# ratan-lab/indelMINER

Measured on AMD Instinct MI355X. Metric: reads/sec through split-read realign+cluster; VCF diff-clean vs reference, higher is better.
Workload: dtype u8/int32; 1 GPU; BASELINE configs[1]: synthetic 1.0 Mb contig per GPU, 100 bp PE reads at 30x, seeded 1-50 bp indels every ~2 kb, BWA-like S/I/D emission; -k 6 -g 0 -s 1000 -n 10 -q 10; pipeline_depth=4, hip_graph=True, parallelism=contig-sharded x1

## Files before the change

### indelminer_amd/csrc/im_rg.hpp

```cpp

#pragma once

#include "im_device.hpp"

namespace im {
namespace {

__device__ __forceinline__ uint32_t ld_u32(const uint8_t* p) { uint32_t v; __builtin_memcpy(&v, p, 4); return v; }

struct RecView {
    const uint8_t* p;
    uint32_t len;
    int32_t tid, pos, mtid, mpos, isize, l_seq;
    uint32_t l_qname, mapq, n_cigar, flag;
    uint32_t o_cigar, o_seq, o_aux;
    uint32_t cig[4];
    bool ok;
};

constexpr int kAuxWin = 24;

__device__ __forceinline__ RecView view_record(const uint8_t* raw, uint32_t off, uint32_t end)
{
    RecView r;
    r.p = raw + off; r.len = end - off; r.ok = false;
    r.tid = r.pos = r.mtid = r.mpos = r.isize = r.l_seq = 0;
    r.l_qname = r.mapq = r.n_cigar = r.flag = 0; r.o_cigar = r.o_seq = r.o_aux = 0;
    r.cig[0] = r.cig[1] = r.cig[2] = r.cig[3] = 0;
    if (end < off || r.len < 32u) return r;
    const uint32_t* c = reinterpret_cast<const uint32_t*>(r.p);
    r.tid = (int32_t)c[0]; r.pos = (int32_t)c[1];
    const uint32_t w2 = c[2], w3 = c[3];
    r.l_qname = w2 & 255u; r.mapq = (w2 >> 8) & 255u;
    r.n_cigar = w3 & 0xFFFFu; r.flag = w3 >> 16;
    r.l_seq = (int32_t)c[4]; r.mtid = (int32_t)c[5]; r.mpos = (int32_t)c[6]; r.isize = (int32_t)c[7];
    if (r.l_seq < 0) return r;
    r.o_cigar = 32u + r.l_qname;
    r.o_seq = r.o_cigar + 4u * r.n_cigar;
    const bool no_qual = (w2 >> 16) == 0xFFFFu;
    const uint64_t o_aux = (uint64_t)r.o_seq + (((uint64_t)r.l_seq + 1u) >> 1) + (no_qual ? 0ull : (uint64_t)r.l_seq);
    if (o_aux > r.len) return r;
    r.o_aux = (uint32_t)o_aux;
    r.ok = true;
    return r;
}

__device__ __forceinline__ int aux_size(uint32_t t)
{
    switch (t) {
    case 'A': case 'c': case 'C': return 1;
    case 's': case 'S': return 2;
    case 'i': case 'I': case 'f': return 4;
    case 'd': return 8;
    default: return 0;
    }
}

struct AuxWin { uint32_t* lds; uint32_t o0; };
__device__ __forceinline__ uint32_t rec_byte(const RecView& r, const AuxWin& w, uint32_t o)
{
    const uint32_t d = o - w.o0;
    return d < (uint32_t)kAuxWin ? reinterpret_cast<const uint8_t*>(w.lds)[d] : r.p[o];
}
__device__ __forceinline__ void aux_slide(const RecView& r, AuxWin& w, uint32_t o)
{
    w.o0 = o;
#pragma unroll
    for (int k = 0; k < kAuxWin / 4; k++) w.lds[k] = ld_u32(r.p + o + 4u * k);
}
__device__ __forceinline__ uint32_t walk_byte(const RecView& r, AuxWin& w, uint32_t o)
{
    if (o - w.o0 >= (uint32_t)kAuxWin) aux_slide(r, w, o);
    return reinterpret_cast<const uint8_t*>(w.lds)[o - w.o0];
}
__device__ __forceinline__ void aux_cover(const RecView& r, AuxWin& w, uint32_t o, uint32_t need)
{
    if (!(o >= w.o0 && o + need <= w.o0 + (uint32_t)kAuxWin)) aux_slide(r, w, o);
}

__device__ __forceinline__ void find_rg_mq(const RecView& r, AuxWin& w, uint32_t& o_rg, uint32_t& o_mq)
{
    o_rg = 0; o_mq = 0;
    uint32_t s = r.o_aux;
    const uint32_t end = r.len;
    while (s + 4u <= end) {
        aux_cover(r, w, s, 8u);
        const uint32_t t0 = rec_byte(r, w, s), t1 = rec_byte(r, w, s + 1), type = rec_byte(r, w, s + 2);
        if (t0 == 'R' && t1 == 'G' && !o_rg) o_rg = s + 2u;
        if (t0 == 'M' && t1 == 'Q' && !o_mq) o_mq = s + 2u;
        if (o_rg && o_mq) return;
        s += 3u;
        if (type == 'Z' || type == 'H') { while (s < end && walk_byte(r, w, s)) s++; s++; }
        else if (type == 'B') {
            if (s + 5u > end) return;
            const int sz = aux_size(rec_byte(r, w, s));
            const uint32_t cnt = rec_byte(r, w, s + 1) | (rec_byte(r, w, s + 2) << 8) | (rec_byte(r, w, s + 3) << 16) | (rec_byte(r, w, s + 4) << 24);
            const uint64_t ns = (uint64_t)s + 5u + (uint64_t)sz * cnt;
            if (ns > end) return;
            s = (uint32_t)ns;
        } else {
            const int sz = aux_size(type);
            if (sz == 0) return;
            s += (uint32_t)sz;
        }
    }
}

struct RgView {
    const int32_t* bin_start; const int32_t* name_off; const int32_t* name_len; const int32_t* range_max; const uint8_t* names;
};
__device__ __forceinline__ RgView rg_view(const uint8_t* blob, int32_t n)
{
    RgView v;
    const int32_t* w = reinterpret_cast<const int32_t*>(blob);
    const int32_t m = n > 0 ? n : 1;
    v.bin_start = w; v.name_off = w + 20; v.name_len = w + 20 + m; v.range_max = w + 20 + 2 * m;
    v.names = blob + 4 * (20 + 3 * m);
    return v;
}

template <typename NameAt>
__device__ __forceinline__ bool rg_lookup(const RgView& T, NameAt name_at, uint32_t len, int32_t& range_max)
{
    uint32_t h = 5381u;
    for (int i = (int)len - 1; i >= 0; i--) h += (h << 5) + (uint32_t)(int32_t)(int8_t)name_at((uint32_t)i);
    const uint32_t bin = h & 15u;
    bool hit = false;
    for (int32_t e = T.bin_start[bin]; e < T.bin_start[bin + 1]; e++) {
        const uint32_t el = (uint32_t)T.name_len[e];
        if (el < len) continue;
        const uint8_t* en = T.names + T.name_off[e];
        bool same = true;
        for (uint32_t i = 0; i < len && same; i++) same = en[i] == name_at(i);
        if (same) { hit = true; range_max = T.range_max[e]; }
    }
    return hit;
}

__device__ __forceinline__ bool rg_tag_range(const RecView& r, AuxWin& w, uint32_t o_rg, const RgView& T, int32_t& range_max)
{
    const uint32_t type = rec_byte(r, w, o_rg);
    bool ok = type == 'Z' || type == 'H';
    if (ok) {
        uint32_t len = 0;
        while (o_rg + 1u + len < r.len) {
            const uint32_t o = o_rg + 1u + len;
            if (o - w.o0 >= (uint32_t)kAuxWin && w.o0 != o_rg) aux_slide(r, w, o_rg);
            if (!rec_byte(r, w, o)) break;
            len++;
        }
        const uint32_t o_name = o_rg + 1u;
        ok = rg_lookup(T, [&](uint32_t k) { return rec_byte(r, w, o_name + k); }, len, range_max);
    }
    return ok;
}

constexpr int kRgLds = 2048;

}
}
```

### indelminer_amd/csrc/im_triage.hip

```cpp

#include "im_device.hpp"
#include "im_rg.hpp"
#include "im_wave.hpp"

#ifdef IM_STAMPS
constexpr int kTriStampCap = 32768;
__device__ unsigned long long im_tri_stamp_rec[kTriStampCap][8];
#define IM_TRI_STAMP_DECL unsigned long long tri_t_[6]; tri_t_[0] = __builtin_amdgcn_s_memtime(); \
                          tri_t_[1] = tri_t_[2] = tri_t_[3] = tri_t_[4] = tri_t_[5] = tri_t_[0];
#define IM_TRI_STAMP(k, v) do { asm volatile("" :: "v"(v)); tri_t_[k] = __builtin_amdgcn_s_memtime(); } while (0)
#define IM_TRI_STAMP_OUT(lane) do { if ((lane) < 6) { const int l_ = (lane); \
        im_tri_stamp_rec[blockIdx.x % kTriStampCap][l_] = l_ == 0 ? tri_t_[0] : l_ == 1 ? tri_t_[1] : l_ == 2 ? tri_t_[2] : l_ == 3 ? tri_t_[3] : l_ == 4 ? tri_t_[4] : tri_t_[5]; } } while (0)
#else
#define IM_TRI_STAMP_DECL
#define IM_TRI_STAMP(k, v)
#define IM_TRI_STAMP_OUT(lane)
#endif

namespace im {
namespace {

constexpr int kTriBlock = 256;
constexpr int kTriGroup = 32;

__device__ __forceinline__ uint32_t ld_u16(const uint8_t* p) { uint16_t v; __builtin_memcpy(&v, p, 2); return v; }


__device__ __forceinline__ uint32_t cigar_word(const RecView& r, uint32_t k)
{
    return k == 0u ? r.cig[0] : k == 1u ? r.cig[1] : k == 2u ? r.cig[2] : k == 3u ? r.cig[3] : ld_u32(r.p + r.o_cigar + 4u * k);
}

__device__ __forceinline__ int32_t aux_int(const RecView& r, const AuxWin& w, uint32_t o)
{
    const uint32_t type = rec_byte(r, w, o);
    if (o + 1u >= r.len) return 0;
    const uint32_t b0 = rec_byte(r, w, o + 1);
    switch (type) {
    case 'c': return (int32_t)(int8_t)b0;
    case 'C': return (int32_t)b0;
    case 's': return (o + 3u <= r.len) ? (int32_t)(int16_t)(b0 | (rec_byte(r, w, o + 2) << 8)) : 0;
    case 'S': return (o + 3u <= r.len) ? (int32_t)(b0 | (rec_byte(r, w, o + 2) << 8)) : 0;
    case 'i': case 'I':
        return (o + 5u <= r.len) ? (int32_t)(b0 | (rec_byte(r, w, o + 2) << 8) | (rec_byte(r, w, o + 3) << 16) | (rec_byte(r, w, o + 4) << 24)) : 0;
    default: return 0;
    }
}


__device__ __forceinline__ bool reaches_new_readaln(const RecView& r)
{
    const uint32_t f = r.flag;
    return r.ok && !(f & (0x100u | 0x200u | 0x400u | 0x800u)) && (f & 0x1u) && (f & 0x2u) && !(f & (0x4u | 0x8u)) && r.tid == r.mtid;
}

__device__ __forceinline__ uint32_t bases_in_cigar_reach(const RecView& r)
{
    uint64_t qtot = 0;
    for (uint32_t i = 0; i < r.n_cigar; i++) {
        const uint32_t cw = cigar_word(r, i), op = cw & 15u;
        if (op == 0u || op == 1u || op == 4u || op == 7u || op == 8u) qtot += cw >> 4;
    }
    const uint64_t avail = 2ull * (r.len - r.o_seq);
    return (uint32_t)(qtot < avail ? qtot : avail);
}

__device__ __forceinline__ uint32_t good_codes(uint32_t x)
{
    const uint32_t c = x - ((x >> 1) & 0x77777777u) - ((x >> 2) & 0x33333333u) - ((x >> 3) & 0x11111111u);
    return (c >> 2) | (c & ~(c >> 1));
}

__device__ __forceinline__ uint32_t first_refused(const uint4& x)
{
    const uint32_t w[4] = { x.x, x.y, x.z, x.w };
    for (uint32_t k = 0; k < 4u; k++) {
        const uint32_t bad = ~good_codes(w[k]) & 0x11111111u;
        if (bad) return 8u * k + ((uint32_t)__builtin_ctz(((bad & 0x0F0F0F0Fu) << 4) | ((bad >> 4) & 0x0F0F0F0Fu)) >> 2);
    }
    return 32u;
}

__device__ __forceinline__ bool all_good(const uint4& x)
{
    return ((good_codes(x.x) & good_codes(x.y) & good_codes(x.z) & good_codes(x.w)) & 0x11111111u) == 0x11111111u;
}

struct BaseSweep {
    uint4 x[8];
    uint32_t lm[8];
    int shift;
};

__device__ __forceinline__ void sweep_issue(BaseSweep& S, const uint8_t* raw, uint32_t so, uint32_t lim, int lane)
{
    S.shift = __ballot(lim > 128u) != 0ull ? 3 : 2;
    const uint32_t sub = (uint32_t)lane & ((1u << S.shift) - 1u);
    const int grp = lane >> S.shift, per_pass = 64 >> S.shift;
#pragma unroll
    for (int j = 0; j < 8; j++) {
        S.lm[j] = 0u; S.x[j] = make_uint4(0x11111111u, 0x11111111u, 0x11111111u, 0x11111111u);
        if (j < (1 << S.shift)) {
            const int src = per_pass * j + grp;
            S.lm[j] = (uint32_t)__shfl((int)lim, src);
            const uint32_t so_j = (uint32_t)__shfl((int)so, src);
            __builtin_memcpy(&S.x[j], raw + (32u * sub < S.lm[j] ? so_j + 16u * sub : 0u), 16);
        }
    }
}

__device__ __forceinline__ void sweep_finish(const BaseSweep& S, const uint8_t* raw, uint32_t so, uint32_t lim, uint32_t* s_fb, int lane)
{
    const uint32_t lanes = 1u << S.shift, sub = (uint32_t)lane & (lanes - 1u);
    const int grp = lane >> S.shift, per_pass = 64 >> S.shift;
#pragma unroll
    for (int j = 0; j < 8; j++) {
        if (j < (1 << S.shift) && 32u * sub < S.lm[j] && !all_good(S.x[j])) {
            const uint32_t idx = 32u * sub + first_refused(S.x[j]);
            if (idx < S.lm[j]) atomicMin(&s_fb[per_pass * j + grp], idx);
        }
    }
    if (__ballot(lim > 256u) != 0ull) {
        for (int j = 0; j < 8; j++) {
            const int src = per_pass * j + grp;
            const uint32_t lm = (uint32_t)__shfl((int)lim, src), so_j = (uint32_t)__shfl((int)so, src);
            for (uint32_t first = 256u + 32u * sub; first < lm; first += 256u) {
                uint4 x; __builtin_memcpy(&x, raw + so_j + (first >> 1), 16);
                if (!all_good(x)) { const uint32_t idx = first + first_refused(x); if (idx < lm) atomicMin(&s_fb[src], idx); }
            }
        }
    }
}

struct Verdict {
    uint32_t cls;
    bool revcomp;
    int32_t range_max;
};

__device__ __forceinline__ Verdict classify(const RecView& r, AuxWin w, const im_triage_params& tp, const RgView& T,
                                            bool generic_ok, int32_t generic_range, uint32_t fb)
{
    Verdict v; v.cls = IM_REC_SKIP; v.revcomp = false; v.range_max = 0;
    if (!r.ok) { v.cls = IM_REC_ERR_LIMIT; return v; }
    const uint32_t flag = r.flag;
    if (flag & (0x100u | 0x200u | 0x400u | 0x800u)) return v;
    const bool aligned = !(flag & 0x4u), mate_aligned = !(flag & 0x8u);
    const bool proper = (flag & 0x2u) != 0, is_rc = (flag & 0x10u) != 0, mate_rc = (flag & 0x20u) != 0;
    if (!(flag & 0x1u)) return v;
    if (aligned && mate_aligned && r.tid != r.mtid) return v;
    v.cls = IM_REC_COUNTED;

    uint32_t o_rg, o_mq;
    find_rg_mq(r, w, o_rg, o_mq);
    if (tp.defer_ranges) {
        if (o_rg) { const uint32_t type = rec_byte(r, w, o_rg); if (!(type == 'Z' || type == 'H')) { v.cls = IM_REC_ERR_RG; return v; } }
        v.range_max = 0;
    } else if (!o_rg) {
        if (!generic_ok) { v.cls = IM_REC_ERR_RG; return v; }
        v.range_max = generic_range;
    } else {
        if (!rg_tag_range(r, w, o_rg, T, v.range_max)) { v.cls = IM_REC_ERR_RG; return v; }
    }

    if (aligned && !mate_aligned) return v;
    if (!aligned && mate_aligned) {
        int32_t mmq = (int32_t)r.mapq;
        if (o_mq) {
            aux_cover(r, w, o_mq, 5u);
            const uint32_t t = rec_byte(r, w, o_mq);
            if (!(t == 'I' || t == 'i' || t == 'C' || t == 'c' || t == 'S' || t == 's')) { v.cls = IM_REC_ERR_MQ; return v; }
            mmq = aux_int(r, w, o_mq);
        }
        if (mmq >= tp.qthreshold) { v.cls = IM_REC_CAND_UNMAPPED; v.revcomp = !mate_rc; }
        return v;
    }
    if (aligned && mate_aligned && proper) {
        const uint32_t lim = bases_in_cigar_reach(r);
        if (fb >= lim) {
            fb = 0xFFFFFFFFu;
            for (uint32_t j = (uint32_t)r.l_seq; j < lim; j++) {
                const uint32_t code = (r.p[r.o_seq + (j >> 1)] >> ((~j & 1u) << 2)) & 15u;
                if (!(code == 1u || code == 2u || code == 4u || code == 8u || code == 15u)) { fb = j; break; }
            }
        }
        uint32_t ndel = 0, nins = 0, nclip = 0; bool three = false;
        uint64_t q = 0;
        for (uint32_t i = 0; i < r.n_cigar; i++) {
            const uint32_t cw = cigar_word(r, i), op = cw & 15u;
            if (op == 3u || op == 5u || op == 6u || op > 8u) { v.cls = (uint64_t)fb < q ? IM_REC_ERR_BASE : IM_REC_ERR_CIGAR; return v; }
            if (op == 0u || op == 1u || op == 4u || op == 7u || op == 8u) q += cw >> 4;
            ndel += op == 2u; nins += op == 1u; nclip += op == 4u;
            if (op == 4u && ((!is_rc && i == r.n_cigar - 1u) || (is_rc && i == 0u))) three = true;
        }
        if (fb != 0xFFFFFFFFu) { v.cls = IM_REC_ERR_BASE; return v; }
        if (ndel + nins + nclip == 0u) return v;
        if ((nclip == 0u || (nclip == 1u && three)) && ndel == 0u && nins == 0u) return v;
        if (o_mq) aux_cover(r, w, o_mq, 5u);
        const int32_t mmq = o_mq ? aux_int(r, w, o_mq) : (int32_t)r.mapq;
        if (mmq >= tp.qthreshold) { v.cls = IM_REC_CAND_PROPER; v.revcomp = is_rc == mate_rc; }
        return v;
    }
    if (aligned && mate_aligned && !proper) {
        const int64_t a = r.isize < 0 ? -(int64_t)r.isize : (int64_t)r.isize;
        const uint32_t a32 = (uint32_t)(r.isize < 0 ? -r.isize : r.isize);
        if (a > (int64_t)v.range_max && a32 < tp.maxpedelsize && is_rc != mate_rc) v.cls = IM_REC_PE;
        return v;
    }
    return v;
}

struct TriageArgs {
    im_dev_records recs;
    im_dev_cands out;
    im_triage_params tp;
    RefDev ref;
    RgTable rg;
    int32_t* depth_diff;
    uint32_t* info;
    int32_t* rmax;
    uint2* blk;
    uint2* wg_base;
    uint32_t* seq_at;
    int32_t* chunk_base;
};

__device__ __forceinline__ uint32_t padded4(int32_t l) { return ((uint32_t)l + 3u) & ~3u; }

constexpr int kClsBlock = 64;
constexpr int kClsLdsBudget = 6400;
constexpr int kDepthWin = 1024;
constexpr int kClsRgLds = 448;
static_assert(kTriBlock % kClsBlock == 0 && kTriGroup % (kTriBlock / kClsBlock) == 0, "an emit workgroup's classify blocks lie in one group");
static_assert(kClsBlock < 512, "a workgroup's candidate, counted and error counts take nine bits each of its packed word");
static_assert(kClsBlock * kAuxWin + kClsBlock * 4 + kDepthWin * 4 + kClsRgLds <= kClsLdsBudget, "classify must fit the hole a realign wave leaves");

__device__ __forceinline__ void wave_lds_order() { __builtin_amdgcn_fence(__ATOMIC_ACQ_REL, "wavefront"); }

__global__ __launch_bounds__(kClsBlock, 6) void triage_classify_kernel(TriageArgs A)
{
    __shared__ uint32_t s_aux[kClsBlock][kAuxWin / 4];
    __shared__ uint32_t s_rg[kClsRgLds / 4];
    __shared__ int32_t s_dd[kDepthWin];
    __shared__ uint32_t s_fb[kClsBlock];
    const int lane = threadIdx.x;
    IM_TRI_STAMP_DECL
    const int64_t i = (int64_t)blockIdx.x * kClsBlock + lane;
    if (A.depth_diff) {
        int4* z = reinterpret_cast<int4*>(s_dd);
#pragma unroll
        for (int k = 0; k < kDepthWin / 4 / kClsBlock; k++) z[lane + k * kClsBlock] = make_int4(0, 0, 0, 0);
    }

    RecView r; r.ok = false; r.l_seq = 0; r.flag = 0; r.n_cigar = 0; r.tid = -1; r.pos = 0; r.o_cigar = 0; r.o_seq = 0; r.p = A.recs.raw; r.len = 0; r.o_aux = 0;
    s_fb[lane] = 0xFFFFFFFFu;
    const bool rg_lds = A.rg.bytes <= kClsRgLds;
    if (rg_lds) for (int k = lane; 4 * k < A.rg.bytes; k += kClsBlock) s_rg[k] = reinterpret_cast<const uint32_t*>(A.rg.blob)[k];
    if (i < A.recs.n) r = view_record(A.recs.raw, A.recs.rec_off[i], A.recs.rec_off[i + 1]);
    IM_TRI_STAMP(1, r.flag);
    const uint32_t sw_lim = reaches_new_readaln(r) ? (uint32_t)r.l_seq : 0u;
    const uint32_t sw_so = sw_lim ? (uint32_t)(r.p - A.recs.raw) + r.o_seq : 0u;
    BaseSweep S;
    sweep_issue(S, A.recs.raw, sw_so, sw_lim, lane);
    if (r.ok) {
#pragma unroll
        for (int k = 0; k < 4; k++) r.cig[k] = ld_u32(r.p + r.o_cigar + 4u * k);
        const uint32_t aux_bytes = r.len - r.o_aux;
#pragma unroll
        for (int k = 0; k < kAuxWin / 4; k++) if (4u * k < aux_bytes) s_aux[lane][k] = ld_u32(r.p + r.o_aux + 4u * k);
    }
    wave_lds_order();
    sweep_finish(S, A.recs.raw, sw_so, sw_lim, s_fb, lane);
    const bool piles = A.depth_diff && r.ok && r.tid >= 0 && r.tid < A.ref.n_contigs && !(r.flag & (0x4u | 0x100u | 0x200u | 0x400u));
    int32_t dd_pos = 0, dd_tid = -1;
    if (A.depth_diff) {
        const uint64_t mp = __ballot(piles);
        const int first = mp ? (int)__builtin_ctzll(mp) : 0;
        const int fp = __shfl(r.pos, first), ft = __shfl(r.tid, first);
        dd_pos = fp < 0 ? 0 : fp; dd_tid = mp ? ft : -1;
    }
    wave_lds_order();
    IM_TRI_STAMP(2, r.cig[3]);
    const RgView T = rg_view(rg_lds ? reinterpret_cast<const uint8_t*>(s_rg) : A.rg.blob, A.rg.n);

    uint32_t cls = IM_REC_SKIP, bytes = 0;
    bool cand = false;
    if (i < A.recs.n) {
        AuxWin w; w.lds = s_aux[lane]; w.o0 = r.o_aux;
        const Verdict v = classify(r, w, A.tp, T, A.rg.generic_ok != 0, A.rg.generic_range, s_fb[lane]);
        cls = v.cls;
        cand = cls == IM_REC_CAND_UNMAPPED || cls == IM_REC_CAND_PROPER;
        if (cand) bytes = padded4(r.l_seq);
        A.info[i] = cls | (v.revcomp ? 0x100u : 0u);
        A.rmax[i] = v.range_max;
        if (A.out.rec_class) A.out.rec_class[i] = (uint8_t)cls;
        if (piles) {
            const int64_t base = A.ref.asc_off[r.tid];
            const int64_t clen = A.ref.len[r.tid];
            const bool here = r.tid == dd_tid;
            int64_t x = r.pos;
            for (uint32_t k = 0; k < r.n_cigar; k++) {
                const uint32_t cw = cigar_word(r, k), op = cw & 15u;
                const int64_t len = cw >> 4;
                if (op == 0u || op == 7u || op == 8u) {
                    int64_t a = x < 0 ? 0 : x, b = x + len > clen ? clen : x + len;
                    if (a < b) {
                        const int64_t ra = a - dd_pos, rb = b - dd_pos;
                        if (here && ra >= 0 && ra < kDepthWin) atomicAdd(&s_dd[ra], 1); else atomicAdd(&A.depth_diff[base + a], 1);
                        if (here && rb >= 0 && rb < kDepthWin) atomicAdd(&s_dd[rb], -1); else atomicAdd(&A.depth_diff[base + b], -1);
                    }
                    x += len;
                } else if (op == 2u || op == 3u) x += len;
            }
        }
    }
    IM_TRI_STAMP(3, cls);
    const uint64_t mc = __ballot(cand);
    uint32_t wb = bytes;
#pragma unroll
    for (int o = 32; o > 0; o >>= 1) wb += (uint32_t)__shfl_xor((int)wb, o);
    const uint64_t mk = __ballot(cls != IM_REC_SKIP), me = __ballot(cls >= IM_REC_ERR_RG);
    wave_lds_order();
    if (A.depth_diff && dd_tid >= 0) {
        int32_t* dst = A.depth_diff + A.ref.asc_off[dd_tid] + dd_pos;
        const int64_t room = (int64_t)A.ref.len[dd_tid] + 1 - dd_pos;
#pragma unroll 4
        for (int k = 0; k < kDepthWin / kClsBlock; k++) {
            const int idx = lane + k * kClsBlock;
            const int32_t v = s_dd[idx];
            if (v != 0 && idx < room) atomicAdd(&dst[idx], v);
        }
    }
    IM_TRI_STAMP(4, wb);
    if (lane == 0) A.blk[blockIdx.x] = make_uint2((uint32_t)__popcll(mc) | ((uint32_t)__popcll(mk) << 9) | ((uint32_t)__popcll(me) << 18), wb);
    IM_TRI_STAMP(5, wb);
    IM_TRI_STAMP_OUT(lane);
}

constexpr int kScanLanes = 256;
constexpr int kScanPerLane = kTriBlock / kClsBlock;
constexpr int kAhead = 8;
static_assert(kScanPerLane == 4, "an emit workgroup's words are two 16-byte loads");
static_assert(kAhead * kScanPerLane == kTriGroup, "a lane's kAhead emit workgroups are one group");
static_assert(kTriGroup * sizeof(uint2) == 256, "blk[] is padded to 256 bytes: whole groups");
static_assert(kScanLanes % 64 == 0 && kScanLanes <= 256, "whole waves, and no wider than fits beside the other streams' workgroups");

__global__ __launch_bounds__(kScanLanes) void triage_scan_kernel(TriageArgs A)
{
    constexpr int kWaves = kScanLanes / 64;
    __shared__ uint2 s_tot[2][kWaves];
    __shared__ uint2 s_ke[kWaves];
    const int t = threadIdx.x, lane = t & 63, wave = t >> 6;
    const int32_t n_blocks = (int32_t)(((int64_t)A.recs.n + kClsBlock - 1) / kClsBlock);
    const int32_t n_emit = (n_blocks + kScanPerLane - 1) / kScanPerLane;
    const int32_t n_groups = (n_blocks + kTriGroup - 1) / kTriGroup;
    const int32_t n_passes = (n_groups + kScanLanes - 1) / kScanLanes;
    const bool fresh = A.tp.restart != 0;
    uint32_t carry_c = fresh ? 0u : (uint32_t)A.out.counters[0], carry_b = fresh ? 0u : (uint32_t)A.out.counters[1];
    const uint32_t chunk_first = carry_c;
    const uint4* src = reinterpret_cast<const uint4*>(A.blk);
    uint4 buf[2 * kAhead];
    auto fetch = [&](int32_t pass) {
        const int64_t g = (int64_t)pass * kScanLanes + t;
        const uint4* p = src + (g < n_groups ? g : (int64_t)n_groups - 1) * (2 * kAhead);
#pragma unroll
        for (int i = 0; i < 2 * kAhead; i++) buf[i] = p[i];
    };
    uint32_t sum_k = 0, sum_e = 0;
    for (int32_t pass = 0; pass < n_passes; pass++) {
        fetch(pass);
        const int64_t g = (int64_t)pass * kScanLanes + t;
        const int64_t left_b = (int64_t)n_blocks - g * kTriGroup, left_e = (int64_t)n_emit - g * kAhead;
        const int nb = left_b < 0 ? 0 : left_b > kTriGroup ? kTriGroup : (int)left_b, ne = left_e < 0 ? 0 : left_e > kAhead ? kAhead : (int)left_e;
        uint32_t oc[kAhead], ob[kAhead], own_c = 0, own_b = 0;
#pragma unroll
        for (int j = 0; j < kAhead; j++) {
            const uint4 d0 = buf[2 * j], d1 = buf[2 * j + 1];
            const uint32_t wx[4] = { d0.x, d0.z, d1.x, d1.z }, wy[4] = { d0.y, d0.w, d1.y, d1.w };
            oc[j] = 0u; ob[j] = 0u;
#pragma unroll
            for (int k = 0; k < kScanPerLane; k++) {
                const bool in = j * kScanPerLane + k < nb;
                const uint32_t x = in ? wx[k] : 0u;
                oc[j] += x & 511u; ob[j] += in ? wy[k] : 0u;
                sum_k += (x >> 9) & 511u; sum_e += (x >> 18) & 511u;
            }
            own_c += oc[j]; own_b += ob[j];
        }
        const uint32_t c = (uint32_t)wave_scan_add((int)own_c, lane), b = (uint32_t)wave_scan_add((int)own_b, lane);
        uint2* tot = s_tot[pass & 1];
        if (lane == 63) tot[wave] = make_uint2(c, b);
        __syncthreads();
        uint32_t front_c = 0, front_b = 0, all_c = 0, all_b = 0;
#pragma unroll
        for (int w = 0; w < kWaves; w++) {
            const uint2 v = tot[w];
            if (w < wave) { front_c += v.x; front_b += v.y; }
            all_c += v.x; all_b += v.y;
        }
        uint32_t at_c = carry_c + front_c + c - own_c, at_b = carry_b + front_b + b - own_b;
#pragma unroll
        for (int j = 0; j < kAhead; j++) {
            if (j < ne) A.wg_base[g * kAhead + j] = make_uint2(at_c, at_b);
            at_c += oc[j]; at_b += ob[j];
        }
        carry_c += all_c; carry_b += all_b;
    }
    sum_k = (uint32_t)wave_sum((int)sum_k); sum_e = (uint32_t)wave_sum((int)sum_e);
    if (lane == 0) s_ke[wave] = make_uint2(sum_k, sum_e);
    __syncthreads();
    if (t == 0) {
        uint32_t k = 0, e = 0;
#pragma unroll
        for (int w = 0; w < kWaves; w++) { k += s_ke[w].x; e += s_ke[w].y; }
        A.chunk_base[0] = (int32_t)chunk_first;
        const int32_t k0 = fresh ? 0 : A.out.counters[2], e0 = fresh ? 0 : A.out.counters[3];
        A.out.counters[0] = (int32_t)carry_c; A.out.counters[1] = (int32_t)carry_b;
        A.out.counters[2] = k0 + (int32_t)k;
        A.out.counters[3] = e0 + (int32_t)e;
        if (fresh) A.out.counters[4] = 0;
    }
}

__device__ __forceinline__ uint32_t base_ascii(uint32_t code)
{
    return code == 1u ? 'A' : code == 2u ? 'C' : code == 4u ? 'G' : code == 8u ? 'T' : code == 15u ? 'N' : 0u;
}
__device__ __forceinline__ uint32_t comp_code(uint32_t c) { return ((c & 1u) << 3) | ((c & 2u) << 1) | ((c & 4u) >> 1) | ((c & 8u) >> 3); }

__global__ __launch_bounds__(kTriBlock) void triage_emit_kernel(TriageArgs A)
{
    __shared__ uint32_t s_cnt[kTriBlock / 64], s_bytes[kTriBlock / 64];
    const int t = threadIdx.x, lane = t & 63, wave = t >> 6;
    const int64_t i = (int64_t)blockIdx.x * kTriBlock + t;
    uint32_t info = 0;
    RecView r; r.ok = false; r.l_seq = 0; r.o_seq = 0; r.p = A.recs.raw;
    if (i < A.recs.n) {
        info = A.info[i];
        const uint32_t cls = info & 255u;
        if (cls == IM_REC_CAND_UNMAPPED || cls == IM_REC_CAND_PROPER) {
            r = view_record(A.recs.raw, A.recs.rec_off[i], A.recs.rec_off[i + 1]);
#pragma unroll
            for (int k = 0; k < 4; k++) r.cig[k] = ld_u32(r.p + r.o_cigar + 4u * k);
        }
    }
    const bool cand = r.ok;
    const uint32_t bytes = cand ? padded4(r.l_seq) : 0u;
    const uint64_t mc = __ballot(cand);
    const uint32_t below = (uint32_t)__popcll(mc & ((1ull << lane) - 1ull));
    uint32_t ib = bytes;
#pragma unroll
    for (int o = 1; o < 64; o <<= 1) { const uint32_t tb = (uint32_t)__shfl_up((int)ib, o); if (lane >= o) ib += tb; }
    if (lane == 63) { s_cnt[wave] = (uint32_t)__popcll(mc); s_bytes[wave] = ib; }
    __syncthreads();
    if (!cand) return;
    uint32_t oc = 0, ob = 0;
    for (int w = 0; w < wave; w++) { oc += s_cnt[w]; ob += s_bytes[w]; }
    const uint2 base = A.wg_base[blockIdx.x];
    const uint32_t ci = base.x + oc + below;
    const uint32_t bo = base.y + ob + ib - bytes;
    const im_dev_batch& B = A.out.batch;
    if (!(ci < (uint32_t)A.out.cap_cand && (uint64_t)bo + bytes + 16u <= (uint64_t)A.out.cap_bases)) {
        atomicAdd(&A.out.counters[4], 1);
        if (ci < (uint32_t)A.out.cap_cand) {
            const_cast<int64_t*>(B.base_off)[ci] = 0;
            const_cast<int32_t*>(B.read_len)[ci] = 0;
            A.seq_at[ci - (uint32_t)A.chunk_base[0]] = 0u;
        }
        return;
    }
    const_cast<int64_t*>(B.base_off)[ci] = (int64_t)bo;
    const_cast<int32_t*>(B.read_len)[ci] = r.l_seq;
    const_cast<int32_t*>(B.tid)[ci] = r.mtid;
    const_cast<int32_t*>(B.anchor)[ci] = r.mpos;
    const_cast<int32_t*>(B.range_max)[ci] = A.rmax[i];
    A.out.cand_rec[ci] = A.recs.rec_base + (int32_t)i;
    A.seq_at[ci - (uint32_t)A.chunk_base[0]] = ((uint32_t)(r.p - A.recs.raw) + r.o_seq) | ((info & 0x100u) ? 0x80000000u : 0u);
    int ne = 0;
    uint32_t err = 0;
    int32_t e_cls[IM_MAX_EV] = { -1, -1, -1, -1 }, e_b1[IM_MAX_EV] = { 0, 0, 0, 0 }, e_b2[IM_MAX_EV] = { 0, 0, 0, 0 };
    if ((info & 255u) == IM_REC_CAND_PROPER) {
        uint32_t tpos = 0, rpos = 0;
        for (uint32_t k = 0; k < r.n_cigar; k++) {
            const uint32_t w = cigar_word(r, k), op = w & 15u;
            if (op == 7u || op == 8u || op == 0u || op == 1u) tpos += w >> 4;
        }
        int32_t refpos = r.pos;
        bool over = false;
        for (uint32_t k = 0; k < r.n_cigar && !err; k++) {
            const uint32_t w = cigar_word(r, k), op = w & 15u, len = w >> 4;
            if (op == 2u || op == 1u) {
                if (rpos > A.tp.ethreshold_vcfcheck && (tpos - rpos) > A.tp.ethreshold_vcfcheck) {
                    const int32_t c = op == 2u ? IM_CLS_DELETION : IM_CLS_INSERTION, x1 = refpos, x2 = op == 2u ? refpos + (int32_t)len : refpos;
                    if (ne == 0) { e_cls[0] = c; e_b1[0] = x1; e_b2[0] = x2; }
                    else if (ne == 1) { e_cls[1] = c; e_b1[1] = x1; e_b2[1] = x2; }
                    else if (ne == 2) { e_cls[2] = c; e_b1[2] = x1; e_b2[2] = x2; }
                    else if (ne == 3) { e_cls[3] = c; e_b1[3] = x1; e_b2[3] = x2; }
                    else over = true;
                    ne += ne < IM_MAX_EV ? 1 : 0;
                }
            } else if (op == 0u || op == 7u || op == 8u) rpos += len;
            else if (op == 4u) { if (!(k == 0u || k == r.n_cigar - 1u)) err = IM_REC_ERR_CLIP; }
            else err = IM_REC_ERR_CIGAR;
            if (op == 0u || op == 7u || op == 8u || op == 2u) refpos += (int32_t)len;
        }
        if (!err && over) err = IM_REC_ERR_LIMIT;
    }
    if (B.ev_cls) {
#pragma unroll
        for (int k = 0; k < IM_MAX_EV; k++) {
            const int64_t sl = (int64_t)ci * IM_MAX_EV + k;
            if (A.out.consumed) A.out.consumed[sl] = 0;
            B.ev_cls[sl] = err ? -1 : e_cls[k];
            B.ev_b1[sl] = err ? 0 : e_b1[k];
            B.ev_b2[sl] = err ? 0 : e_b2[k];
        }
    }
    if (err) {
        A.info[i] = (info & ~255u) | err;
        if (A.out.rec_class) A.out.rec_class[i] = (uint8_t)err;
        atomicAdd(&A.out.counters[3], 1);
    }
}

__global__ __launch_bounds__(256) void triage_decode_kernel(TriageArgs A)
{
    const int sub = threadIdx.x >> 5, l32 = threadIdx.x & 31;
    const int32_t c0 = A.chunk_base[0];
    const int32_t c1 = min(A.out.counters[0], A.out.cap_cand);
    for (int32_t ci = c0 + (int32_t)blockIdx.x * 8 + sub; ci < c1; ci += (int32_t)gridDim.x * 8) {
        const uint32_t at = A.seq_at[ci - c0];
        const bool rc = (at & 0x80000000u) != 0;
        const uint8_t* seq = A.recs.raw + (at & 0x7FFFFFFFu);
        const int32_t L = A.out.batch.read_len[ci];
        uint8_t* dst = const_cast<uint8_t*>(A.out.batch.bases) + A.out.batch.base_off[ci];
        bool bad = false;
        for (int32_t p0 = 4 * l32; p0 < (int32_t)padded4(L); p0 += 128) {
            const int32_t n_here = min(4, L - p0);
            const int32_t qlo = rc ? L - p0 - n_here : p0;
            const uint32_t packed = rc ? ld_u32(seq + (qlo >> 1)) : ld_u16(seq + (p0 >> 1));
            const int32_t b0 = qlo >> 1;
            uint32_t word = 0;
#pragma unroll
            for (int j = 0; j < 4; j++) {
                if (j >= n_here) break;
                const int32_t q = rc ? L - 1 - p0 - j : p0 + j;
                const uint32_t byte = (packed >> (8 * ((q >> 1) - b0))) & 255u;
                uint32_t code = (q & 1) ? (byte & 15u) : (byte >> 4);
                if (rc) code = comp_code(code);
                const uint32_t ch = base_ascii(code);
                bad |= ch == 0u;
                word |= ch << (8 * j);
            }
            *reinterpret_cast<uint32_t*>(dst + p0) = word;
        }
        const uint64_t mb = __ballot(bad);
        const uint32_t half = (uint32_t)(mb >> (32 * ((threadIdx.x >> 5) & 1)));
        if (half != 0u && l32 == 0) {
            const int32_t rec = A.out.cand_rec[ci] - A.recs.rec_base;
            if ((A.info[rec] & 255u) < IM_REC_ERR_RG) {
                if (A.out.rec_class) A.out.rec_class[rec] = (uint8_t)IM_REC_ERR_BASE;
                atomicAdd(&A.out.counters[3], 1);
            }
        }
    }
}

}

constexpr size_t kTriFixed = 256;

size_t triage_scratch_bytes(int32_t n_records)
{
    const size_t n = (size_t)(n_records > 0 ? n_records : 1);
    const size_t emits = (n + kTriBlock - 1) / kTriBlock;
    auto up = [](size_t x) { return (x + 255) / 256 * 256; };
    return up(n * 4) + up(n * 4) + up(emits * (kTriBlock / kClsBlock) * 8) + up(emits * 8) + up(n * 4) + kTriFixed;
}

size_t triage_scratch_zero_offset(int32_t n_records, size_t* bytes)
{
    (void)n_records;
    *bytes = kTriFixed;
    return 0;
}

#ifdef IM_STAMPS
extern "C" int im_debug_tri_stamps_read(unsigned long long* out, int n_rec, int reset)
{
    if (n_rec < 0 || n_rec > kTriStampCap) return -1;
    hipError_t e = hipDeviceSynchronize();
    if (e == hipSuccess) e = hipMemcpyFromSymbol(out, HIP_SYMBOL(im_tri_stamp_rec), (size_t)n_rec * 64);
    void* sym = nullptr;
    if (e == hipSuccess && reset) e = hipGetSymbolAddress(&sym, HIP_SYMBOL(im_tri_stamp_rec));
    if (e == hipSuccess && reset) e = hipMemset(sym, 0, sizeof(im_tri_stamp_rec));
    return e == hipSuccess ? 0 : -1;
}
#endif

hipError_t launch_triage(const RefDev& ref, const RgTable& rg, int32_t* depth_diff, const im_triage_params& tp,
                         const im_dev_records& recs, const im_dev_cands& out, void* scratch, hipStream_t stream)
{
    if (recs.n <= 0) return hipSuccess;
    const size_t n = (size_t)recs.n;
    const int blocks = (int)((n + kTriBlock - 1) / kTriBlock), cls_blocks = (int)((n + kClsBlock - 1) / kClsBlock);
    auto up = [](size_t x) { return (x + 255) / 256 * 256; };
    TriageArgs A;
    A.recs = recs; A.out = out; A.tp = tp; A.ref = ref; A.rg = rg;
    A.depth_diff = tp.want_depth ? depth_diff : nullptr;
    char* s = static_cast<char*>(scratch);
    A.chunk_base = reinterpret_cast<int32_t*>(s); s += 256;
    A.info = reinterpret_cast<uint32_t*>(s); s += up(n * 4);
    A.rmax = reinterpret_cast<int32_t*>(s); s += up(n * 4);
    A.blk = reinterpret_cast<uint2*>(s); s += up((size_t)blocks * (kTriBlock / kClsBlock) * 8);
    A.wg_base = reinterpret_cast<uint2*>(s); s += up((size_t)blocks * 8);
    A.seq_at = reinterpret_cast<uint32_t*>(s);
    hipLaunchKernelGGL(triage_classify_kernel, dim3(cls_blocks), dim3(kClsBlock), 0, stream, A);
    hipLaunchKernelGGL(triage_scan_kernel, dim3(1), dim3(kScanLanes), 0, stream, A);
    hipLaunchKernelGGL(triage_emit_kernel, dim3(blocks), dim3(kTriBlock), 0, stream, A);
    int dgrid = (int)((n + 63) / 64);
    if (dgrid > 16384) dgrid = 16384;
    hipLaunchKernelGGL(triage_decode_kernel, dim3(dgrid), dim3(256), 0, stream, A);
    return hipGetLastError();
}

}
```

Baseline: 6.873 billion reads/s.

## Flatten triage classification into wave-uniform predicated passes over CIGAR and aux tags

Replaces the per-lane early-return classify() with a branch-free pipeline: one CIGAR pass, bounded by the wave-wide maximum op count, that gathers query length, refused ops, clip facts and depth-diff pile-ups together. The aux tag walk and the slow MQ and RG paths are rewritten as ballot-guarded loops so divergent lanes step in lockstep, and the aux/cigar prefetch is made unconditional with split load/store phases. The aim is less SIMT divergence and fewer repeated CIGAR traversals. In exchange every lane runs work predicated off for its record, and the depth range arithmetic now uses biased 32-bit values.

```diff
diff --git a/indelminer_amd/csrc/im_rg.hpp b/indelminer_amd/csrc/im_rg.hpp
--- a/indelminer_amd/csrc/im_rg.hpp
+++ b/indelminer_amd/csrc/im_rg.hpp
@@ -47,13 +47,7 @@
 
 __device__ __forceinline__ int aux_size(uint32_t t)
 {
-    switch (t) {
-    case 'A': case 'c': case 'C': return 1;
-    case 's': case 'S': return 2;
-    case 'i': case 'I': case 'f': return 4;
-    case 'd': return 8;
-    default: return 0;
-    }
+    return (t == 'A' || t == 'c' || t == 'C') ? 1 : (t == 's' || t == 'S') ? 2 : (t == 'i' || t == 'I' || t == 'f') ? 4 : t == 'd' ? 8 : 0;
 }
 
 struct AuxWin { uint32_t* lds; uint32_t o0; };
@@ -65,44 +59,68 @@
 __device__ __forceinline__ void aux_slide(const RecView& r, AuxWin& w, uint32_t o)
 {
     w.o0 = o;
+    uint32_t v[kAuxWin / 4];
 #pragma unroll
-    for (int k = 0; k < kAuxWin / 4; k++) w.lds[k] = ld_u32(r.p + o + 4u * k);
+    for (int k = 0; k < kAuxWin / 4; k++) v[k] = ld_u32(r.p + o + 4u * k);
+#pragma unroll
+    for (int k = 0; k < kAuxWin / 4; k++) w.lds[k] = v[k];
 }
 __device__ __forceinline__ uint32_t walk_byte(const RecView& r, AuxWin& w, uint32_t o)
 {
     if (o - w.o0 >= (uint32_t)kAuxWin) aux_slide(r, w, o);
     return reinterpret_cast<const uint8_t*>(w.lds)[o - w.o0];
 }
+__device__ __forceinline__ bool aux_covers(const AuxWin& w, uint32_t o, uint32_t need)
+{
+    return o >= w.o0 && o + need <= w.o0 + (uint32_t)kAuxWin;
+}
 __device__ __forceinline__ void aux_cover(const RecView& r, AuxWin& w, uint32_t o, uint32_t need)
 {
-    if (!(o >= w.o0 && o + need <= w.o0 + (uint32_t)kAuxWin)) aux_slide(r, w, o);
+    if (!aux_covers(w, o, need)) aux_slide(r, w, o);
+}
+__device__ __forceinline__ uint32_t win_byte(const AuxWin& w, uint32_t o, bool on)
+{
+    return reinterpret_cast<const uint8_t*>(w.lds)[on ? o - w.o0 : 0u];
 }
 
-__device__ __forceinline__ void find_rg_mq(const RecView& r, AuxWin& w, uint32_t& o_rg, uint32_t& o_mq)
+__device__ __forceinline__ void find_rg_mq(const RecView& r, AuxWin& w, uint32_t& o_rg, uint32_t& o_mq, bool walk = true)
 {
     o_rg = 0; o_mq = 0;
     uint32_t s = r.o_aux;
     const uint32_t end = r.len;
-    while (s + 4u <= end) {
-        aux_cover(r, w, s, 8u);
-        const uint32_t t0 = rec_byte(r, w, s), t1 = rec_byte(r, w, s + 1), type = rec_byte(r, w, s + 2);
-        if (t0 == 'R' && t1 == 'G' && !o_rg) o_rg = s + 2u;
-        if (t0 == 'M' && t1 == 'Q' && !o_mq) o_mq = s + 2u;
-        if (o_rg && o_mq) return;
+    bool on = walk && s + 4u <= end;
+    while (__ballot(on) != 0ull) {
+        const bool move = on && !aux_covers(w, s, 8u);
+        if (__ballot(move) != 0ull) { if (move) aux_slide(r, w, s); }
+        const uint32_t t0 = win_byte(w, s, on), t1 = win_byte(w, s + 1u, on), type = win_byte(w, s + 2u, on);
+        if (on && t0 == 'R' && t1 == 'G' && !o_rg) o_rg = s + 2u;
+        if (on && t0 == 'M' && t1 == 'Q' && !o_mq) o_mq = s + 2u;
+        on = on && !(o_rg && o_mq);
         s += 3u;
-        if (type == 'Z' || type == 'H') { while (s < end && walk_byte(r, w, s)) s++; s++; }
-        else if (type == 'B') {
-            if (s + 5u > end) return;
-            const int sz = aux_size(rec_byte(r, w, s));
-            const uint32_t cnt = rec_byte(r, w, s + 1) | (rec_byte(r, w, s + 2) << 8) | (rec_byte(r, w, s + 3) << 16) | (rec_byte(r, w, s + 4) << 24);
-            const uint64_t ns = (uint64_t)s + 5u + (uint64_t)sz * cnt;
-            if (ns > end) return;
-            s = (uint32_t)ns;
-        } else {
-            const int sz = aux_size(type);
-            if (sz == 0) return;
-            s += (uint32_t)sz;
+        const bool str = on && (type == 'Z' || type == 'H'), arr = on && type == 'B';
+        const uint32_t sz = (uint32_t)aux_size(type);
+        if (on && !str && !arr) { on = sz != 0u; s += sz; }
+        if (__ballot(str) != 0ull) {
+            bool go = str;
+            for (;;) {
+                go = go && s < end;
+                const bool mv = go && s - w.o0 >= (uint32_t)kAuxWin;
+                if (__ballot(mv) != 0ull) { if (mv) aux_slide(r, w, s); }
+                go = go && win_byte(w, s, go) != 0u;
+                if (__ballot(go) == 0ull) break;
+                s += go ? 1u : 0u;
+            }
+            s += str ? 1u : 0u;
         }
+        if (__ballot(arr) != 0ull) {
+            const bool hdr = arr && s + 5u <= end;
+            const uint32_t esz = (uint32_t)aux_size(win_byte(w, s, hdr));
+            const uint32_t cnt = win_byte(w, s + 1u, hdr) | (win_byte(w, s + 2u, hdr) << 8) | (win_byte(w, s + 3u, hdr) << 16) | (win_byte(w, s + 4u, hdr) << 24);
+            const uint64_t ns = (uint64_t)s + 5u + (uint64_t)esz * cnt;
+            const bool fits = hdr && ns <= end;
+            if (arr) { on = fits; s = fits ? (uint32_t)ns : s; }
+        }
+        on = on && s + 4u <= end;
     }
 }
 
diff --git a/indelminer_amd/csrc/im_triage.hip b/indelminer_amd/csrc/im_triage.hip
--- a/indelminer_amd/csrc/im_triage.hip
+++ b/indelminer_amd/csrc/im_triage.hip
@@ -54,17 +54,6 @@
     return r.ok && !(f & (0x100u | 0x200u | 0x400u | 0x800u)) && (f & 0x1u) && (f & 0x2u) && !(f & (0x4u | 0x8u)) && r.tid == r.mtid;
 }
 
-__device__ __forceinline__ uint32_t bases_in_cigar_reach(const RecView& r)
-{
-    uint64_t qtot = 0;
-    for (uint32_t i = 0; i < r.n_cigar; i++) {
-        const uint32_t cw = cigar_word(r, i), op = cw & 15u;
-        if (op == 0u || op == 1u || op == 4u || op == 7u || op == 8u) qtot += cw >> 4;
-    }
-    const uint64_t avail = 2ull * (r.len - r.o_seq);
-    return (uint32_t)(qtot < avail ? qtot : avail);
-}
-
 __device__ __forceinline__ uint32_t good_codes(uint32_t x)
 {
     const uint32_t c = x - ((x >> 1) & 0x77777777u) - ((x >> 2) & 0x33333333u) - ((x >> 3) & 0x11111111u);
@@ -132,84 +121,17 @@
     }
 }
 
-struct Verdict {
-    uint32_t cls;
-    bool revcomp;
-    int32_t range_max;
+constexpr uint32_t kOpsRefused = 0xFE68u, kOpsQuery = 0x193u, kOpsMatch = 0x181u, kOpsRef = 0x18Du;
+
+__device__ __forceinline__ uint32_t add_sat(uint32_t a, uint32_t b) { const uint32_t s = a + b; return s < a ? 0xFFFFFFFFu : s; }
+
+struct CigarFacts {
+    uint32_t seen;
+    uint32_t qtot;
+    uint32_t q0;
+    uint32_t nclip;
+    bool three;
 };
-
-__device__ __forceinline__ Verdict classify(const RecView& r, AuxWin w, const im_triage_params& tp, const RgView& T,
-                                            bool generic_ok, int32_t generic_range, uint32_t fb)
-{
-    Verdict v; v.cls = IM_REC_SKIP; v.revcomp = false; v.range_max = 0;
-    if (!r.ok) { v.cls = IM_REC_ERR_LIMIT; return v; }
-    const uint32_t flag = r.flag;
-    if (flag & (0x100u | 0x200u | 0x400u | 0x800u)) return v;
-    const bool aligned = !(flag & 0x4u), mate_aligned = !(flag & 0x8u);
-    const bool proper = (flag & 0x2u) != 0, is_rc = (flag & 0x10u) != 0, mate_rc = (flag & 0x20u) != 0;
-    if (!(flag & 0x1u)) return v;
-    if (aligned && mate_aligned && r.tid != r.mtid) return v;
-    v.cls = IM_REC_COUNTED;
-
-    uint32_t o_rg, o_mq;
-    find_rg_mq(r, w, o_rg, o_mq);
-    if (tp.defer_ranges) {
-        if (o_rg) { const uint32_t type = rec_byte(r, w, o_rg); if (!(type == 'Z' || type == 'H')) { v.cls = IM_REC_ERR_RG; return v; } }
-        v.range_max = 0;
-    } else if (!o_rg) {
-        if (!generic_ok) { v.cls = IM_REC_ERR_RG; return v; }
-        v.range_max = generic_range;
-    } else {
-        if (!rg_tag_range(r, w, o_rg, T, v.range_max)) { v.cls = IM_REC_ERR_RG; return v; }
-    }
-
-    if (aligned && !mate_aligned) return v;
-    if (!aligned && mate_aligned) {
-        int32_t mmq = (int32_t)r.mapq;
-        if (o_mq) {
-            aux_cover(r, w, o_mq, 5u);
-            const uint32_t t = rec_byte(r, w, o_mq);
-            if (!(t == 'I' || t == 'i' || t == 'C' || t == 'c' || t == 'S' || t == 's')) { v.cls = IM_REC_ERR_MQ; return v; }
-            mmq = aux_int(r, w, o_mq);
-        }
-        if (mmq >= tp.qthreshold) { v.cls = IM_REC_CAND_UNMAPPED; v.revcomp = !mate_rc; }
-        return v;
-    }
-    if (aligned && mate_aligned && proper) {
-        const uint32_t lim = bases_in_cigar_reach(r);
-        if (fb >= lim) {
-            fb = 0xFFFFFFFFu;
-            for (uint32_t j = (uint32_t)r.l_seq; j < lim; j++) {
-                const uint32_t code = (r.p[r.o_seq + (j >> 1)] >> ((~j & 1u) << 2)) & 15u;
-                if (!(code == 1u || code == 2u || code == 4u || code == 8u || code == 15u)) { fb = j; break; }
-            }
-        }
-        uint32_t ndel = 0, nins = 0, nclip = 0; bool three = false;
-        uint64_t q = 0;
-        for (uint32_t i = 0; i < r.n_cigar; i++) {
-            const uint32_t cw = cigar_word(r, i), op = cw & 15u;
-            if (op == 3u || op == 5u || op == 6u || op > 8u) { v.cls = (uint64_t)fb < q ? IM_REC_ERR_BASE : IM_REC_ERR_CIGAR; return v; }
-            if (op == 0u || op == 1u || op == 4u || op == 7u || op == 8u) q += cw >> 4;
-            ndel += op == 2u; nins += op == 1u; nclip += op == 4u;
-            if (op == 4u && ((!is_rc && i == r.n_cigar - 1u) || (is_rc && i == 0u))) three = true;
-        }
-        if (fb != 0xFFFFFFFFu) { v.cls = IM_REC_ERR_BASE; return v; }
-        if (ndel + nins + nclip == 0u) return v;
-        if ((nclip == 0u || (nclip == 1u && three)) && ndel == 0u && nins == 0u) return v;
-        if (o_mq) aux_cover(r, w, o_mq, 5u);
-        const int32_t mmq = o_mq ? aux_int(r, w, o_mq) : (int32_t)r.mapq;
-        if (mmq >= tp.qthreshold) { v.cls = IM_REC_CAND_PROPER; v.revcomp = is_rc == mate_rc; }
-        return v;
-    }
-    if (aligned && mate_aligned && !proper) {
-        const int64_t a = r.isize < 0 ? -(int64_t)r.isize : (int64_t)r.isize;
-        const uint32_t a32 = (uint32_t)(r.isize < 0 ? -r.isize : r.isize);
-        if (a > (int64_t)v.range_max && a32 < tp.maxpedelsize && is_rc != mate_rc) v.cls = IM_REC_PE;
-        return v;
-    }
-    return v;
-}
-
 struct TriageArgs {
     im_dev_records recs;
     im_dev_cands out;
@@ -253,66 +175,157 @@
     }
 
     RecView r; r.ok = false; r.l_seq = 0; r.flag = 0; r.n_cigar = 0; r.tid = -1; r.pos = 0; r.o_cigar = 0; r.o_seq = 0; r.p = A.recs.raw; r.len = 0; r.o_aux = 0;
+    r.mtid = -1; r.isize = 0; r.mapq = 0;
     s_fb[lane] = 0xFFFFFFFFu;
     const bool rg_lds = A.rg.bytes <= kClsRgLds;
     if (rg_lds) for (int k = lane; 4 * k < A.rg.bytes; k += kClsBlock) s_rg[k] = reinterpret_cast<const uint32_t*>(A.rg.blob)[k];
-    if (i < A.recs.n) r = view_record(A.recs.raw, A.recs.rec_off[i], A.recs.rec_off[i + 1]);
+    const bool valid = i < A.recs.n;
+    if (valid) r = view_record(A.recs.raw, A.recs.rec_off[i], A.recs.rec_off[i + 1]);
     IM_TRI_STAMP(1, r.flag);
-    const uint32_t sw_lim = reaches_new_readaln(r) ? (uint32_t)r.l_seq : 0u;
+    const bool pp = reaches_new_readaln(r);
+    const uint32_t sw_lim = pp ? (uint32_t)r.l_seq : 0u;
     const uint32_t sw_so = sw_lim ? (uint32_t)(r.p - A.recs.raw) + r.o_seq : 0u;
     BaseSweep S;
     sweep_issue(S, A.recs.raw, sw_so, sw_lim, lane);
-    if (r.ok) {
-#pragma unroll
-        for (int k = 0; k < 4; k++) r.cig[k] = ld_u32(r.p + r.o_cigar + 4u * k);
-        const uint32_t aux_bytes = r.len - r.o_aux;
-#pragma unroll
-        for (int k = 0; k < kAuxWin / 4; k++) if (4u * k < aux_bytes) s_aux[lane][k] = ld_u32(r.p + r.o_aux + 4u * k);
+    {
+        const uint8_t* pc = r.ok ? r.p + r.o_cigar : A.recs.raw;
+        const uint8_t* pa = r.ok ? r.p + r.o_aux : A.recs.raw;
+        uint32_t av[kAuxWin / 4];
+#pragma unroll
+        for (int k = 0; k < 4; k++) r.cig[k] = ld_u32(pc + 4u * k);
+#pragma unroll
+        for (int k = 0; k < kAuxWin / 4; k++) av[k] = ld_u32(pa + 4u * k);
+#pragma unroll
+        for (int k = 0; k < kAuxWin / 4; k++) s_aux[lane][k] = av[k];
     }
     wave_lds_order();
     sweep_finish(S, A.recs.raw, sw_so, sw_lim, s_fb, lane);
     const bool piles = A.depth_diff && r.ok && r.tid >= 0 && r.tid < A.ref.n_contigs && !(r.flag & (0x4u | 0x100u | 0x200u | 0x400u));
     int32_t dd_pos = 0, dd_tid = -1;
+    int64_t pl_base = 0;
+    uint32_t pl_end = 0;
     if (A.depth_diff) {
         const uint64_t mp = __ballot(piles);
         const int first = mp ? (int)__builtin_ctzll(mp) : 0;
         const int fp = __shfl(r.pos, first), ft = __shfl(r.tid, first);
         dd_pos = fp < 0 ? 0 : fp; dd_tid = mp ? ft : -1;
+        if (mp) {
+            const int32_t t = piles ? r.tid : dd_tid;
+            pl_base = A.ref.asc_off[t];
+            pl_end = (uint32_t)A.ref.len[t] ^ 0x80000000u;
+        }
     }
     wave_lds_order();
     IM_TRI_STAMP(2, r.cig[3]);
     const RgView T = rg_view(rg_lds ? reinterpret_cast<const uint8_t*>(s_rg) : A.rg.blob, A.rg.n);
 
-    uint32_t cls = IM_REC_SKIP, bytes = 0;
-    bool cand = false;
-    if (i < A.recs.n) {
-        AuxWin w; w.lds = s_aux[lane]; w.o0 = r.o_aux;
-        const Verdict v = classify(r, w, A.tp, T, A.rg.generic_ok != 0, A.rg.generic_range, s_fb[lane]);
-        cls = v.cls;
-        cand = cls == IM_REC_CAND_UNMAPPED || cls == IM_REC_CAND_PROPER;
-        if (cand) bytes = padded4(r.l_seq);
-        A.info[i] = cls | (v.revcomp ? 0x100u : 0u);
-        A.rmax[i] = v.range_max;
+    const uint32_t flag = r.flag;
+    const bool aligned = !(flag & 0x4u), mate_aligned = !(flag & 0x8u), both = aligned && mate_aligned;
+    const bool proper = (flag & 0x2u) != 0, is_rc = (flag & 0x10u) != 0, mate_rc = (flag & 0x20u) != 0;
+    const bool counted = r.ok && !(flag & (0x100u | 0x200u | 0x400u | 0x800u)) && (flag & 0x1u) && !(both && r.tid != r.mtid);
+
+    CigarFacts cf; cf.seen = 0u; cf.qtot = 0u; cf.q0 = 0u; cf.nclip = 0u; cf.three = false;
+    {
+        const uint32_t nc = (pp || piles) ? r.n_cigar : 0u;
+        const uint32_t nmax = (uint32_t)wave_max((int)nc);
+        const uint32_t three_at = is_rc ? 0u : r.n_cigar - 1u;
+        const bool here = r.tid == dd_tid;
+        uint32_t u = (uint32_t)r.pos ^ 0x80000000u;
+        auto op_step = [&](uint32_t k, uint32_t cw) {
+            const uint32_t bit = k < nc ? 1u << (cw & 15u) : 0u, len = cw >> 4;
+            if ((bit & kOpsRefused) && !(cf.seen & kOpsRefused)) cf.q0 = cf.qtot;
+            cf.seen |= bit;
+            cf.qtot = add_sat(cf.qtot, (bit & kOpsQuery) ? len : 0u);
+            cf.nclip += (bit >> 4) & 1u;
+            cf.three = cf.three || ((bit & 16u) && k == three_at);
+            const uint32_t ue = add_sat(u, (bit & kOpsRef) ? len : 0u);
+            const uint32_t au = u > 0x80000000u ? u : 0x80000000u, bu = ue < pl_end ? ue : pl_end;
+            if (piles && (bit & kOpsMatch) && au < bu) {
+                const int32_t a = (int32_t)(au ^ 0x80000000u), b = (int32_t)(bu ^ 0x80000000u);
+                const uint32_t ra = (uint32_t)(a - dd_pos), rb = (uint32_t)(b - dd_pos);
+                if (here && ra < (uint32_t)kDepthWin) atomicAdd(&s_dd[ra], 1); else atomicAdd(&A.depth_diff[pl_base + a], 1);
+                if (here && rb < (uint32_t)kDepthWin) atomicAdd(&s_dd[rb], -1); else atomicAdd(&A.depth_diff[pl_base + b], -1);
+            }
+            u = ue;
+        };
+#pragma unroll
+        for (uint32_t k = 0; k < 4u; k++) if (k < nmax) op_step(k, r.cig[k]);
+        for (uint32_t k = 4u; k < nmax; k++) {
+            uint32_t cw = 0u;
+            if (k < nc) cw = ld_u32(r.p + r.o_cigar + 4u * k);
+            op_step(k, cw);
+        }
+    }
+
+    AuxWin w; w.lds = s_aux[lane]; w.o0 = r.o_aux;
+    uint32_t o_rg, o_mq;
+    find_rg_mq(r, w, o_rg, o_mq, counted);
+    const bool defer = A.tp.defer_ranges != 0;
+    const bool has_rg = counted && o_rg != 0u;
+    const bool generic = counted && !has_rg && !defer;
+    bool rg_err = generic && A.rg.generic_ok == 0;
+    int32_t rmax = (generic && A.rg.generic_ok != 0) ? A.rg.generic_range : 0;
+    if (__ballot(has_rg) != 0ull) {
+        if (has_rg) {
+            if (defer) { const uint32_t type = rec_byte(r, w, o_rg); rg_err = !(type == 'Z' || type == 'H'); }
+            else { int32_t rm = 0; if (rg_tag_range(r, w, o_rg, T, rm)) rmax = rm; else rg_err = true; }
+        }
+    }
+    const bool live = counted && !rg_err;
+    const bool um = live && !aligned && mate_aligned;
+    const bool ppl = live && both && proper;
+    const bool pe = live && both && !proper;
+
+    const uint32_t avail = 2u * (r.len - r.o_seq);
+    const uint32_t lim = cf.qtot < avail ? cf.qtot : avail;
+    uint32_t fb = s_fb[lane];
+    fb = fb >= lim ? 0xFFFFFFFFu : fb;
+    const bool behind = ppl && fb == 0xFFFFFFFFu && lim > (uint32_t)r.l_seq;
+    if (__ballot(behind) != 0ull) {
+        if (behind) {
+            for (uint32_t j = (uint32_t)r.l_seq; j < lim; j++) {
+                const uint32_t code = (r.p[r.o_seq + (j >> 1)] >> ((~j & 1u) << 2)) & 15u;
+                if (!(code == 1u || code == 2u || code == 4u || code == 8u || code == 15u)) { fb = j; break; }
+            }
+        }
+    }
+    const uint32_t pp_err = (cf.seen & kOpsRefused) ? (fb < cf.q0 ? IM_REC_ERR_BASE : IM_REC_ERR_CIGAR) : fb != 0xFFFFFFFFu ? IM_REC_ERR_BASE : 0u;
+    const bool variant = (cf.seen & 6u) != 0u || cf.nclip > 1u || (cf.nclip == 1u && !cf.three);
+
+    const bool need_mq = o_mq != 0u && (um || (ppl && pp_err == 0u && variant));
+    const bool mq_in = need_mq && aux_covers(w, o_mq, 2u);
+    const uint32_t mq_type = win_byte(w, o_mq, mq_in), mq_byte = win_byte(w, o_mq + 1u, mq_in);
+    const bool mq_fast = mq_in && mq_type == 'C';
+    int32_t mmq = mq_fast ? (int32_t)mq_byte : (int32_t)r.mapq;
+    bool mq_err = false;
+    const bool mq_slow = need_mq && !mq_fast;
+    if (__ballot(mq_slow) != 0ull) {
+        if (mq_slow) {
+            aux_cover(r, w, o_mq, 5u);
+            const uint32_t t = rec_byte(r, w, o_mq);
+            mq_err = um && !(t == 'I' || t == 'i' || t == 'C' || t == 'c' || t == 'S' || t == 's');
+            mmq = aux_int(r, w, o_mq);
+        }
+    }
+    const bool mq_pass = mmq >= A.tp.qthreshold;
+
+    const uint32_t a32 = r.isize < 0 ? 0u - (uint32_t)r.isize : (uint32_t)r.isize;
+    const bool pe_hit = (rmax < 0 || a32 > (uint32_t)rmax) && a32 < A.tp.maxpedelsize && is_rc != mate_rc;
+    uint32_t cls = !valid ? IM_REC_SKIP : !r.ok ? IM_REC_ERR_LIMIT : !counted ? IM_REC_SKIP : rg_err ? IM_REC_ERR_RG : IM_REC_COUNTED;
+    bool revcomp = false;
+    if (um) { cls = mq_err ? IM_REC_ERR_MQ : mq_pass ? IM_REC_CAND_UNMAPPED : IM_REC_COUNTED; revcomp = !mq_err && mq_pass && !mate_rc; }
+    if (ppl) {
+        const bool hit = pp_err == 0u && variant && mq_pass;
+        cls = pp_err != 0u ? pp_err : hit ? IM_REC_CAND_PROPER : IM_REC_COUNTED;
+        revcomp = hit && is_rc == mate_rc;
+    }
+    if (pe && pe_hit) cls = IM_REC_PE;
+    const bool cand = cls == IM_REC_CAND_UNMAPPED || cls == IM_REC_CAND_PROPER;
+    const uint32_t bytes = cand ? padded4(r.l_seq) : 0u;
+    if (valid) {
+        A.info[i] = cls | (revcomp ? 0x100u : 0u);
+        A.rmax[i] = rmax;
         if (A.out.rec_class) A.out.rec_class[i] = (uint8_t)cls;
-        if (piles) {
-            const int64_t base = A.ref.asc_off[r.tid];
-            const int64_t clen = A.ref.len[r.tid];
-            const bool here = r.tid == dd_tid;
-            int64_t x = r.pos;
-            for (uint32_t k = 0; k < r.n_cigar; k++) {
-                const uint32_t cw = cigar_word(r, k), op = cw & 15u;
-                const int64_t len = cw >> 4;
-                if (op == 0u || op == 7u || op == 8u) {
-                    int64_t a = x < 0 ? 0 : x, b = x + len > clen ? clen : x + len;
-                    if (a < b) {
-                        const int64_t ra = a - dd_pos, rb = b - dd_pos;
-                        if (here && ra >= 0 && ra < kDepthWin) atomicAdd(&s_dd[ra], 1); else atomicAdd(&A.depth_diff[base + a], 1);
-                        if (here && rb >= 0 && rb < kDepthWin) atomicAdd(&s_dd[rb], -1); else atomicAdd(&A.depth_diff[base + b], -1);
-                    }
-                    x += len;
-                } else if (op == 2u || op == 3u) x += len;
-            }
-        }
     }
     IM_TRI_STAMP(3, cls);
     const uint64_t mc = __ballot(cand);
```

Measured after the change: 7.123 billion reads/s, median of 6. 3.6% higher.
